# p2004dr/visual-slam

Hardware: AMD Instinct MI355X
Metric: frames/sec (extract+match+pose) at 640×480, 2000 ORB, 1/2/4/8 MI355X (higher is better)
Workload: dtype u8

## Files before the change

include/vslam_amd.h:

```cpp
#ifndef VSLAM_AMD_H
#define VSLAM_AMD_H

#include <stddef.h>
#include <stdint.h>

#ifdef __cplusplus
extern "C" {
#endif

#define MO_ABI_VERSION 5
int mo_abi_version(void);

#define MO_OK 0
#define MO_ERR_ARG (-1)
#define MO_ERR_HIP (-2)
#define MO_ERR_CAPACITY (-3)
#define MO_ERR_UNSUPPORTED (-4)

#define MO_ORDER_LIBSTDCXX 0
#define MO_ORDER_MSVC 1

typedef struct mo_ctx mo_ctx;

typedef struct {
// ... 198 lines not shown

int mo_dev_status(mo_ctx*, int32_t flags[4]);

int mo_stage_times(mo_ctx*, const char*** names, float* ms, int cap);
int mo_stage_times_back(mo_ctx*, int back, const char*** names, float* ms, int cap);

int mo_host_times(mo_ctx*, double us[4]);
int mo_set_host_timing(mo_ctx*, int on);

int mo_dbg_pyramid_level(mo_ctx*, const mo_orb_params*, const uint8_t* gray, int w, int h, int level, int blurred,
                         uint8_t* out , int* lw, int* lh);
int mo_dbg_fast_level(mo_ctx*, const mo_orb_params*, const uint8_t* gray, int w, int h, int level,
                      int32_t* xys , int cap, int* n);
int mo_dbg_min_eigen(mo_ctx*, const uint8_t* gray, int w, int h, float* eig );
int mo_dbg_set_poison(mo_ctx*, int byte );
int mo_dbg_retain_best(mo_ctx*, const float* resp, int n, int n_points, int select_order, int32_t* order, int* n_out);

#ifdef __cplusplus
}
#endif
#endif
```

visual-slam_amd/csrc/api.hip:

```cpp
#include <algorithm>
#include <cmath>
#include <cstring>
#include <vector>

#include "common.h"

static inline int* host_flags(mo_ctx* c) { return mo_host_flags(c); }

extern "C" int mo_set_host_timing(mo_ctx* c, int on) {
    if (!c) return MO_ERR_ARG;
    c->host_timing = on != 0;
    return MO_OK;
}

extern "C" int mo_host_times(mo_ctx* c, double us[4]) {
    if (!c || !us) return MO_ERR_ARG;
    for (int i = 0; i < 4; i++) us[i] = c->host_us[i];
    return MO_OK;
}

static bool grow_fin_slots(mo_ctx* c, int levels);

static int check_flags(mo_ctx* c) {
    int f[4] = {0, 0, 0, 0};
// ... 21 lines not shown
                   mo_keypoint* d_kps, uint8_t* d_desc, int cap, int32_t* d_counts, int host_call) {
    int rc = mo_build_plan(c, p, w, h, batch);
    if (rc) return rc;
    if (cap < 1) return mo_fail(c, MO_ERR_ARG, "cap must be >= 1");
    c->flags_cur = host_call ? host_flags(c) : c->d_flags;
    if (host_call == 1) HIPCHK(c, hipMemsetAsync(host_flags(c), 0, 4 * sizeof(int), c->stream));
    if (c->poison >= 0) {
        HIPCHK(c, hipMemsetAsync(c->d_pyr, c->poison, (size_t)c->batch_alloc * c->plan.pyr_stride, c->stream));
        HIPCHK(c, hipMemsetAsync(c->d_blur, c->poison, (size_t)c->batch_alloc * c->plan.blur_stride, c->stream));
    }
    if (host_call) mo_stage_mark(c, "h2d");
    else mo_stage_begin(c);
    const int blur_margin = (c->plan.edge_threshold - 19) & ~3, pyr_margin = std::max(blur_margin - 4, 0);
    if (batch <= MO_FS_MAX_BATCH && c->fs_ok) {
        if ((rc = orb_launch_front_single(c, d_gray, batch, d_desc != nullptr))) return rc;
        mo_stage_mark(c, "pyramid");
        if (d_desc) mo_stage_mark(c, "blur");
    } else {
        if ((rc = orb_launch_pyramid(c, d_gray, batch, c->plan.nlevels, pyr_margin))) return rc;
        mo_stage_mark(c, "pyramid");
        if (d_desc) {
            if ((rc = orb_launch_blur(c, d_gray, batch, c->plan.nlevels, blur_margin))) return rc;
            mo_stage_mark(c, "blur");
        }
    }
    if ((rc = orb_launch_fast(c, d_gray, batch))) return rc;
    mo_stage_mark(c, "fast_nms");
    if ((rc = orb_launch_select(c, d_gray, batch))) return rc;
    mo_stage_mark(c, "select_harris");
    if ((rc = orb_launch_describe(c, d_gray, batch, d_kps, d_desc, cap, d_counts))) return rc;
// ... 359 lines not shown
    const int nk = hn[65];
    if (hn[64] != n || nk < 0 || nk > n) return mo_fail(c, MO_ERR_HIP, "grid corner counts disagree between host and device");
    *n_xy = n; *n_kept = nk;
    std::memcpy(kept_idx, ho + (o_kept - o_out), (size_t)nk * sizeof(int32_t));
    std::memcpy(desc, ho + (o_desc - o_out), (size_t)nk * 32);
    mo_slot_commit(c, slot, nk);
    return MO_OK;
}

extern "C" int mo_dbg_set_poison(mo_ctx* c, int byte) {
    if (!c) return MO_ERR_ARG;
    c->poison = byte < 0 ? -1 : (byte & 255);
    return MO_OK;
}

extern "C" int mo_dbg_min_eigen(mo_ctx* c, const uint8_t* gray, int w, int h, float* eig) {
    if (!c) return MO_ERR_ARG;
    HIPCHK(c, hipSetDevice(c->device));
    return gftt_run(c, gray, w, h, w, 1, 64, nullptr, nullptr, eig);
}

extern "C" int mo_match_knn2_ratio(mo_ctx* c, const uint8_t* q, int nq, const uint8_t* t, int nt, const double* ratio,
                                   int batch, int32_t* train_idx, int32_t* dist, uint8_t* pass) {
    if (!c) return MO_ERR_ARG;
    if (nq < 0 || nt < 0 || batch < 1) return mo_fail(c, MO_ERR_ARG, "bad sizes");
    if (nq == 0) return MO_OK;
    if (!q || !train_idx || !dist || !pass || (nt > 0 && !t)) return mo_fail(c, MO_ERR_ARG, "NULL argument");
    HIPCHK(c, hipSetDevice(c->device));
    HostClock clk(c);
    size_t qb = (size_t)batch * nq * 32, tb = (size_t)batch * std::max(nt, 1) * 32, n = (size_t)batch * nq;
// ... 336 lines not shown
        mo_stage_mark(c, "two_view");
    }
    return MO_OK;
}

extern "C" int mo_dbg_pyramid_level(mo_ctx* c, const mo_orb_params* p, const uint8_t* gray, int w, int h, int level,
                                    int blurred, uint8_t* out, int* lw, int* lh) {
    if (!c) return MO_ERR_ARG;
    HIPCHK(c, hipSetDevice(c->device));
    int rc = mo_build_plan(c, p, w, h, 1);
    if (rc) return rc;
    if (level < 0 || level >= c->plan.nlevels) return mo_fail(c, MO_ERR_ARG, "level out of range");
    const uint8_t* d_gray = nullptr;
    if ((rc = stage_images(c, gray, w, h, w, 1, 1, &d_gray))) return rc;
    const bool fused = (blurred & 2) != 0;
    blurred &= 1;
    if (fused) {
        if (!c->fs_ok) return mo_fail(c, MO_ERR_UNSUPPORTED, std::string("the single-frame pyramid kernel does not cover this geometry: ") + c->fs_why);
        HIPCHK(c, hipMemsetAsync(c->d_pyr, 0xA5, (size_t)c->plan.pyr_stride, c->stream));
        HIPCHK(c, hipMemsetAsync(c->d_blur, 0xA5, (size_t)c->plan.blur_stride, c->stream));
        if ((rc = orb_launch_front_single(c, d_gray, 1, 1))) return rc;
    } else if ((rc = orb_launch_pyramid(c, d_gray, 1, c->plan.nlevels, 0))) return rc;
    const LevelInfo& v = c->plan.lv[level];
    *lw = v.w; *lh = v.h;
    if (blurred) {
        if (!fused && (rc = orb_launch_blur(c, d_gray, 1, c->plan.nlevels, 0))) return rc;
        HIPCHK(c, hipMemcpy2DAsync(out, v.w, c->d_blur + v.boff, v.bpitch, v.w, v.h, hipMemcpyDeviceToHost, c->stream));
    } else {
        const uint8_t* src = level == 0 ? d_gray : c->d_pyr + v.off;
        HIPCHK(c, hipMemcpy2DAsync(out, v.w, src, v.pitch, v.w, v.h, hipMemcpyDeviceToHost, c->stream));
    }
    HIPCHK(c, hipStreamSynchronize(c->stream));
    return MO_OK;
}

extern "C" int mo_dbg_fast_level(mo_ctx* c, const mo_orb_params* p, const uint8_t* gray, int w, int h, int level,
                                 int32_t* xys, int cap, int* n) {
    if (!c) return MO_ERR_ARG;
    HIPCHK(c, hipSetDevice(c->device));
    int rc = mo_build_plan(c, p, w, h, 1);
    if (rc) return rc;
// ... 44 lines not shown
```

visual-slam_amd/csrc/common.h:

```cpp
#pragma once
#include <hip/hip_runtime.h>
#include <chrono>
#include <stdint.h>
#include <string>
#include <vector>

#include "../../include/vslam_amd.h"

#define MO_MAX_LEVELS 12
#define MO_HALF_PATCH 15
#define MO_STRIP_ROWS 8
#ifndef MO_STRIP_ROWS_LATENCY
#define MO_STRIP_ROWS_LATENCY 2
#endif
#define SEL_MAXSTRIPS 2047

struct LevelInfo {
    int w, h, pitch;
    int off;
    int bpitch, boff;
    float scale;
    int quota;
    int bx0, by0, bw, bh;
    uint32_t inv_bw;
    int strip_rows;
    int nstrips;
    int strip_cap;
    int strip_base;
    int cand_off;
    int cand_cap;
// ... 55 lines not shown

    uint8_t* d_in = nullptr;       size_t d_in_bytes = 0;
    uint8_t* d_gray = nullptr;     size_t d_gray_bytes = 0;
    uint8_t* d_pyr = nullptr;
    uint8_t* d_blur = nullptr;
    uint32_t* d_cand = nullptr;
    int* d_strip_cnt = nullptr;
    uint64_t* d_scratch = nullptr;
    size_t scratch_stride = 0;
    FinalKp* d_fin = nullptr;
    int* d_fin_cnt = nullptr;
    uint32_t* d_tile_tab[2] = {nullptr, nullptr};
    int tile_cum[2][MO_MAX_LEVELS + 1] = {};
    int tile_margin = 0;
    uint32_t* d_fs_tab = nullptr; int fs_tiles = 0, fs_stride = 0, fs_lds = 0; bool fs_ok = false; int fs_geom[10] = {}; const char* fs_why = "";
    uint32_t* d_strip_tab = nullptr; int n_strip_tab = 0;
    uint32_t* d_dtile_tab = nullptr; int n_dtiles = 0, dtile_icw_off = 0;
    int* d_dtodo = nullptr; size_t dtodo_bytes = 0;
    int* d_flags = nullptr;
    int* flags_cur = nullptr;
    unsigned lds_attr_done = 0;
    mo_keypoint* d_kps = nullptr; uint8_t* d_desc = nullptr; int* d_counts = nullptr; int out_cap = 0, out_batch = 0;
    mo_keypoint* d_slot_kps = nullptr; uint8_t* d_slot_desc = nullptr; int32_t* d_slot_cnt = nullptr; int32_t* d_slot_ids = nullptr;
    int slot_cap = 0, slot_cur = -1;
    uint64_t slot_token[MO_RESULT_SLOTS] = {}; int slot_n[MO_RESULT_SLOTS] = {}; uint64_t token_next = 1, last_token = 0;
    bool host_timing = false;
    uint8_t* d_mq = nullptr; uint8_t* d_mt = nullptr; int32_t* d_midx = nullptr; int32_t* d_mdist = nullptr;
    uint8_t* d_mpass = nullptr; size_t m_q_bytes = 0, m_t_bytes = 0, m_n = 0;
    uint2* d_match_part = nullptr; size_t match_part_bytes = 0;
    void* d_tv = nullptr; size_t tv_bytes = 0;
// ... 56 lines not shown
uint64_t mo_slot_commit(mo_ctx* c, int slot, int n);
uint8_t* mo_stage_dev(mo_ctx* c);
void mo_copy_out_launch(mo_ctx* c, const void* d_src, void* h_dst_dev, size_t bytes);

void mo_stage_begin(mo_ctx* c);
void mo_stage_mark(mo_ctx* c, const char* name);

int mo_build_plan(mo_ctx* c, const mo_orb_params* p, int w, int h, int batch);

int orb_launch_gray(mo_ctx* c, const uint8_t* d_bgr, int w, int h, int batch, uint8_t* d_gray);
int orb_launch_ingest(mo_ctx* c, const uint8_t* src_mapped, int w, int h, int ch, uint8_t* d_gray, int* flags_clear);
int orb_launch_pyramid(mo_ctx* c, const uint8_t* d_gray, int batch, int nlevels, int margin);
#define MO_FS_MAX_BATCH 2
int fs_build(mo_ctx* c);
int orb_launch_front_single(mo_ctx* c, const uint8_t* d_gray, int batch, int want_blur);
void mo_linear_coeffs(int srcsize, int dstsize, std::vector<int>& ofs, std::vector<int>& c1);
int orb_launch_blur(mo_ctx* c, const uint8_t* d_gray, int batch, int nlevels, int margin);
int orb_launch_fast(mo_ctx* c, const uint8_t* d_gray, int batch, int level_lo = 0, int level_hi = MO_MAX_LEVELS);
int orb_launch_select(mo_ctx* c, const uint8_t* d_gray, int batch, int level_lo = 0, int level_hi = MO_MAX_LEVELS);
int orb_launch_describe(mo_ctx* c, const uint8_t* d_gray, int batch, mo_keypoint* d_kps, uint8_t* d_desc, int cap,
                        int* d_counts);
int orb_launch_describe_given(mo_ctx* c, const uint8_t* d_gray, const mo_keypoint* d_kps, int n, uint8_t* d_desc, const int* d_n = nullptr,
                              int batch = 1, int n_stride = 0);
int gftt_records_launch(mo_ctx* c, const float* d_xy, int* d_cell_n, int per_cell, int w, int h, int edge, mo_keypoint* d_rec,
                        int32_t* d_kept, int rec_stride, int32_t* d_counts_out, int batch, int32_t* d_kbase = nullptr);
int orb_launch_describe_cells(mo_ctx* c, const mo_keypoint* d_kps, const int32_t* d_kbase, uint8_t* d_desc, int cap, int batch);
int orb_launch_retain_probe(mo_ctx* c, const float* d_resp, int n, int n_points, int order, int32_t* d_order,
                            int* d_nout);
int match_launch_pairs(mo_ctx* c, const uint8_t* d_q, const uint8_t* d_t, size_t q_stride, size_t t_stride,
                       const int32_t* d_counts, const int32_t* d_qf, const int32_t* d_tf, int nq_fixed, int nt_fixed,
// ... 32 lines not shown
```

visual-slam_amd/csrc/ctx.hip:

```cpp
#include <algorithm>
#include <cmath>
#include <cstring>
#include <vector>

#include <cstdlib>

#include "common.h"

int mo_fail(mo_ctx* c, int code, const std::string& msg) {
    if (c) c->err = msg;
    return code;
}

static std::string g_create_err;

static inline int cv_round_f(float v) { return (int)lrintf(v); }
static inline int cv_round_d(double v) { return (int)lrint(v); }
static inline int align_up(int v, int a) { return (v + a - 1) / a * a; }

extern "C" int mo_abi_version(void) { return MO_ABI_VERSION; }

extern "C" int mo_device_count(void) {
    int n = 0;
    if (hipGetDeviceCount(&n) != hipSuccess) return 0;
// ... 36 lines not shown
    hipMemset(c->d_flags, 0, 8 * sizeof(int));
    c->flags_cur = c->d_flags;
    return c;
}

static void free_plan_buffers(mo_ctx* c) {
    for (int L = 0; L < MO_MAX_LEVELS; L++) {
        ResizeTab& t = c->rtab[L];
        if (t.xpk) hipFree(t.xpk);
        t = ResizeTab();
    }
    void* bufs[] = {c->d_pyr, c->d_blur, c->d_cand, c->d_strip_cnt, c->d_scratch, c->d_fin, c->d_fin_cnt, c->d_tile_tab[0], c->d_tile_tab[1], c->d_strip_tab, c->d_dtile_tab};
    c->d_dtile_tab = nullptr; c->n_dtiles = 0;
    if (c->d_fs_tab) hipFree(c->d_fs_tab);
    c->d_fs_tab = nullptr; c->fs_ok = false;
    for (void* b : bufs) if (b) hipFree(b);
    c->d_tile_tab[0] = c->d_tile_tab[1] = nullptr; c->d_strip_tab = nullptr; c->n_strip_tab = 0;
    c->d_pyr = c->d_blur = nullptr; c->d_cand = nullptr; c->d_strip_cnt = nullptr; c->d_scratch = nullptr;
    c->d_fin = nullptr; c->d_fin_cnt = nullptr;
    c->batch_alloc = 0;
    c->plan_valid = false;
}

extern "C" void mo_destroy(mo_ctx* c) {
    if (!c) return;
    hipSetDevice(c->device);
    hipDeviceSynchronize();
    mo_comm_destroy(c);
    free_plan_buffers(c);
    void* bufs[] = {c->d_in, c->d_gray, c->d_flags, c->d_kps, c->d_desc, c->d_counts, c->d_mq, c->d_mt,
// ... 241 lines not shown
    }

    size_t B = (size_t)batch;
    HIPCHK(c, hipMalloc((void**)&c->d_pyr, B * P.pyr_stride));
    HIPCHK(c, hipMalloc((void**)&c->d_blur, B * P.blur_stride));
    HIPCHK(c, hipMalloc((void**)&c->d_cand, B * P.cand_stride * sizeof(uint32_t)));
    HIPCHK(c, hipMalloc((void**)&c->d_strip_cnt, B * P.strips_per_frame * sizeof(int)));
    HIPCHK(c, hipMalloc((void**)&c->d_scratch, B * c->scratch_stride * sizeof(uint64_t)));
    if (hipMalloc((void**)&c->d_fin, B * P.fin_stride * sizeof(FinalKp)) != hipSuccess)
        return mo_fail(c, MO_ERR_HIP, "hipMalloc of the final-keypoint slots failed: " + std::to_string(B * P.fin_stride * sizeof(FinalKp)) +
                                          " bytes (" + std::to_string(batch) + " frames x " + std::to_string(P.fin_stride) + " slots; slots grow with response ties)");
    HIPCHK(c, hipMalloc((void**)&c->d_fin_cnt, B * MO_MAX_LEVELS * sizeof(int)));
    {
        const int rc_fs = fs_build(c);
        if (rc_fs) return rc_fs;
    }
    c->batch_alloc = batch;
    c->plan_params = *p;
    c->plan_valid = true;
    c->fin_slack_dirty = false;
    return MO_OK;
}
```

visual-slam_amd/csrc/orb_kernels.hip:

```cpp
#include <cstring>

#include "common.h"
#include "select_replay.h"

__constant__ __attribute__((aligned(16))) int8_t c_pattern[256 * 4] = {
#include "orb_pattern.inc"
};

#define WAVE 64

__device__ __forceinline__ int reflect101(int p, int len) {
    if (len == 1) return 0;
    while (p < 0 || p >= len) p = p < 0 ? -p : 2 * len - 2 - p;
    return p;
}

__device__ __forceinline__ void xcd_map(uint32_t lin, uint32_t per, uint32_t inv_per, uint32_t batch, int& frame, int& item) {
    const uint32_t b8 = batch & ~7u, cut = per * b8;
    const bool head = lin < cut;
    const uint32_t n = head ? lin >> 3 : lin - cut;
    const uint32_t q = inv_per ? __umulhi(n, inv_per) : n;
    item = (int)(n - q * per);
    frame = (int)(head ? (lin & 7u) + 8u * q : b8 + q);
}

__device__ __forceinline__ const uint8_t* level_ptr(const Plan& P, int L, const uint8_t* gray, const uint8_t* pyr,
                                                    int frame) {
    return L == 0 ? gray + (size_t)frame * P.w * P.h : pyr + (size_t)frame * P.pyr_stride + P.lv[L].off;
}

__global__ void k_gray(const uint8_t* __restrict__ bgr, uint8_t* __restrict__ gray, size_t npx) {
    size_t i = (size_t)blockIdx.x * blockDim.x + threadIdx.x;
    if (i >= npx) return;
    int b = bgr[3 * i], g = bgr[3 * i + 1], r = bgr[3 * i + 2];
    gray[i] = (uint8_t)((b * 3735 + g * 19235 + r * 9798 + (1 << 14)) >> 15);
}

int orb_launch_gray(mo_ctx* c, const uint8_t* d_bgr, int w, int h, int batch, uint8_t* d_gray) {
// ... 1470 lines not shown
```

visual-slam_amd/vslam_amd/__init__.py:

```python
import ctypes as C
import os
import weakref

import numpy as np

_PKG_ROOT = os.path.dirname(os.path.dirname(os.path.abspath(__file__)))
LIB_PATH = os.environ.get("VSLAM_AMD_LIB") or os.path.join(_PKG_ROOT, "libvslam_amd.so")

MO_OK, MO_ERR_ARG, MO_ERR_HIP, MO_ERR_CAPACITY, MO_ERR_UNSUPPORTED = 0, -1, -2, -3, -4
ABI_VERSION = 5
ORDER_LIBSTDCXX, ORDER_MSVC = 0, 1

KP_DTYPE = np.dtype([("x", "<f4"), ("y", "<f4"), ("size", "<f4"), ("angle", "<f4"), ("response", "<f4"),
                     ("octave", "<i4"), ("class_id", "<i4")])
assert KP_DTYPE.itemsize == 28


class NativeUnavailable(RuntimeError):
    pass


class NativeError(RuntimeError):
    def __init__(self, code, msg):
        super().__init__("libvslam_amd error %d: %s" % (code, msg))
# ... 61 lines not shown
SIGNATURES = {
    "mo_create": (_vp, [_i, _i, _i, _i]),
    "mo_destroy": (None, [_vp]),
    "mo_last_error": (C.c_char_p, [_vp]),
    "mo_set_stream": (_i, [_vp, _vp]),
    "mo_set_stream_null": (_i, [_vp]),
    "mo_sync": (_i, [_vp]),
    "mo_device_count": (_i, []),
    "mo_abi_version": (_i, []),
    "mo_orb_detect_compute": (_i, [_vp, _vp, _vp, _i, _i, _i, _i, _i, _vp, _vp, _i, _vp]),
    "mo_orb_compute": (_i, [_vp, _vp, _vp, _i, _i, _i, _i, _vp, _i, _vp, _vp, _vp]),
    "mo_orb_grid_good_features": (_i, [_vp, _vp, _i, _i, _i, _i, _i, _vp, _vp]),
    "mo_orb_grid_detect_compute": (_i, [_vp, _vp, _vp, _i, _i, _i, _i, _i, _vp, _vp, _vp, _vp, _vp]),
    "mo_dbg_min_eigen": (_i, [_vp, _vp, _i, _i, _vp]),
    "mo_dbg_set_poison": (_i, [_vp, _i]),
    "mo_undistort": (_i, [_vp, _vp, _i, _i, _i, _i, _vp, _vp, _vp]),
    "mo_dev_undistort": (_i, [_vp, _vp, _i, _i, _i, _i, _vp, _vp, _vp]),
    "mo_match_knn2_ratio": (_i, [_vp, _vp, _i, _vp, _i, _vp, _i, _vp, _vp, _vp]),
    "mo_init_two_view": (_i, [_vp, _vp, _vp, _i, _vp, _d, _d, _i, C.c_uint64, _vp, _vp, _vp, _vp, _vp, _vp, _vp]),
    "mo_recover_pose": (_i, [_vp, _vp, _vp, _vp, _i, _vp, _vp, _vp, _vp, _vp, _vp, _vp]),
    "mo_find_fundamental": (_i, [_vp, _vp, _vp, _i, _d, _d, _i, C.c_uint64, _vp, _vp, _vp]),
    "mo_track_pair": (_i, [_vp, _vp, _i, _vp, _vp, _i, _vp, _i, _i, _d, _d, _vp, _d, _i, C.c_uint64, _vp, _vp, _vp, _vp, _vp, _vp, _vp,
                           _vp]),
    "mo_triangulate_points": (_i, [_vp, _vp, _vp, _vp, _vp, _i, _vp]),
    "mo_dev_frontend_batch": (_i, [_vp, _vp, _vp]),
    "mo_dev_orb_detect_compute": (_i, [_vp, _vp, _vp, _i, _i, _i, _vp, _vp, _i, _vp]),
    "mo_dev_match_pairs": (_i, [_vp, _vp, _vp, _i, _vp, _vp, _i, _d, _vp, _vp, _vp]),
    "mo_dev_status": (_i, [_vp, _vp]),
    "mo_stream_create": (_vp, [_vp, _vp, _vp]),
    "mo_stream_destroy": (None, [_vp]),
# ... 436 lines not shown
```

Before: 108,200.

## Add banded batched fused pyramid+blur kernel keeping levels in LDS

Adds a new kernel that builds the whole image pyramid and Gaussian blur for each horizontal band of a frame inside LDS. Each workgroup handles one band and recomputes halo rows across levels, replacing the separate per-level resize and blur launches for large batches. A heuristic (fb_pays) turns it on only when there are enough workgroups to keep the CUs busy. The cost is redundant halo computation and one workgroup per CU because of the large LDS footprint.

```diff
diff --git a/include/vslam_amd.h b/include/vslam_amd.h
--- a/include/vslam_amd.h
+++ b/include/vslam_amd.h
@@ -236,6 +236,7 @@
                       int32_t* xys , int cap, int* n);
 int mo_dbg_min_eigen(mo_ctx*, const uint8_t* gray, int w, int h, float* eig );
 int mo_dbg_set_poison(mo_ctx*, int byte );
+int mo_dbg_set_front_batch(mo_ctx*, int on);
 int mo_dbg_retain_best(mo_ctx*, const float* resp, int n, int n_points, int select_order, int32_t* order, int* n_out);
 
 #ifdef __cplusplus
diff --git a/profiles/front_batch_model.py b/profiles/front_batch_model.py
--- /dev/null
+++ b/profiles/front_batch_model.py
@@ -0,0 +1,100 @@
+#!/usr/bin/env python3
+import argparse
+import math
+
+CUS, SIMDS, GHZ = 256, 4, 2.4
+FAST, SLOW = 2.26, 4.5
+LDS_CU = 160 * 1024
+RESIZE_Q = (22, 28)
+BLUR_ROW = (5, 14)
+BLUR_OUT = (6, 16)
+K = 8
+MAX_RECOMPUTE = 0.4
+
+
+def cv_round(x):
+    return int(math.floor(x + 0.5))
+
+
+def linear_ofs(src, dst):
+    scale = src / dst
+    ofs = []
+    for v in range(dst):
+        f = scale * (v + 0.5) - 0.5
+        i = math.floor(f)
+        ofs.append(0 if i < 0 else min(i, src - 1))
+    return ofs
+
+
+def reflect(p, n):
+    while p < 0 or p >= n:
+        p = -p if p < 0 else 2 * n - 2 - p
+    return p
+
+
+def model(w, h, nl, sf, nb, batch, budget):
+    W = [cv_round(w / sf ** L) for L in range(nl)]
+    H = [cv_round(h / sf ** L) for L in range(nl)]
+    yo = [None] + [linear_ofs(H[L - 1], H[L]) for L in range(1, nl)]
+    pw = [((x + 3) & ~3) + 12 for x in W]
+    qr = [((x + 6) >> 2) + 1 for x in W]
+    xtot = sum(4 * qr[L] for L in range(1, nl))
+    own_rows = [0] * nl
+    eys = []
+    ht = hb = 0
+    for b in range(nb):
+        ey = [None] * nl
+        for L in range(nl - 1, -1, -1):
+            o0, o1 = b * H[L] // nb, (b + 1) * H[L] // nb
+            rows = [reflect(y, H[L]) for y in range(o0 - 3, o1 + 3)]
+            lo, hi = min(rows), max(rows)
+            if L + 1 < nl:
+                n0, n1 = ey[L + 1]
+                lo = min(lo, yo[L + 1][n0]); hi = max(hi, min(yo[L + 1][n1 - 1] + 1, H[L] - 1))
+            ey[L] = (lo, hi + 1)
+            own_rows[L] += o1 - o0
+            if L == 0:
+                ht, hb = max(ht, o0 - lo), max(hb, hi + 1 - o1)
+        eys.append(ey)
+    ext_rows = [0] * nl
+    lds_max = 0
+    for b, ey in enumerate(eys):
+        o0, o1 = b * H[0] // nb, (b + 1) * H[0] // nb
+        ey[0] = (max(o0 - ht, 0), min(o1 + hb, H[0]))
+        for L in range(nl):
+            ext_rows[L] += ey[L][1] - ey[L][0]
+        buf = [max((pw[L] * (ey[L][1] - ey[L][0]) + 15) & ~15 for L in range(par, nl, 2)) for par in (0, 1)]
+        ytot = (sum(ey[L][1] - ey[L][0] for L in range(1, nl)) + 3) & ~3
+        lds_max = max(lds_max, sum(buf) + 4 * (xtot + ytot))
+    wg_cu = LDS_CU // lds_max if lds_max <= budget else 0
+    wg_cu = min(wg_cu, 1)
+    quads = lambda L, rows: rows * qr[L] if L else rows * (pw[L] - 12) // 4
+    res_tasks = sum(quads(L, ext_rows[L]) for L in range(1, nl)) / 64
+    bq = lambda L, rows: rows * (pw[L] - 12) // 4
+    blur_rows = sum(bq(L, own_rows[L] * (K + 6) // K) for L in range(nl)) / 64
+    blur_out = sum(bq(L, own_rows[L]) for L in range(nl)) / 64
+    cyc = sum(n * c for (n, c) in [(RESIZE_Q[0] * res_tasks, FAST), (RESIZE_Q[1] * res_tasks, SLOW),
+                                   (BLUR_ROW[0] * blur_rows, FAST), (BLUR_ROW[1] * blur_rows, SLOW),
+                                   (BLUR_OUT[0] * blur_out, FAST), (BLUR_OUT[1] * blur_out, SLOW)])
+    issue_ms = cyc * batch / (CUS * SIMDS) / (GHZ * 1e6)
+    read0 = ext_rows[0] * w
+    wbytes = sum(W[L] * H[L] for L in range(1, nl)) + sum(W[L] * H[L] for L in range(nl))
+    return dict(nb=nb, band0=h // nb, halo0=(ht, hb), recompute=[round(ext_rows[L] / H[L] - 1, 3) for L in range(nl)], lds_kb=round(lds_max / 1024, 1),
+                wg_per_cu=wg_cu, mb_per_step=round((read0 + wbytes) * batch / 1e6, 1), hbm_ms=round((read0 + wbytes) * batch / 6.29e9, 3),
+                issue_ms=round(issue_ms, 3), wgs=nb * batch)
+
+
+if __name__ == "__main__":
+    ap = argparse.ArgumentParser()
+    ap.add_argument("--w", type=int, default=640); ap.add_argument("--h", type=int, default=480)
+    ap.add_argument("--levels", type=int, default=8); ap.add_argument("--scale", type=float, default=1.2)
+    ap.add_argument("--batch", type=int, default=256); ap.add_argument("--budget-kb", type=float, default=158)
+    a = ap.parse_args()
+    budget = a.budget_kb * 1024
+    taken = False
+    for nb in (2, 3, 4, 5, 6, 8, 10, 12, 16, 21):
+        m = model(a.w, a.h, a.levels, a.scale, nb, a.batch, budget)
+        fits = m["lds_kb"] * 1024 <= budget
+        mark = ("  <- fb_build" if m["recompute"][0] <= MAX_RECOMPUTE else "  <- fits, refused by fb_build (halo bound)") if not taken and fits else ""
+        taken = taken or bool(mark)
+        print(m, mark)
diff --git a/visual-slam_amd/csrc/api.hip b/visual-slam_amd/csrc/api.hip
--- a/visual-slam_amd/csrc/api.hip
+++ b/visual-slam_amd/csrc/api.hip
@@ -59,6 +59,10 @@
     const int blur_margin = (c->plan.edge_threshold - 19) & ~3, pyr_margin = std::max(blur_margin - 4, 0);
     if (batch <= MO_FS_MAX_BATCH && c->fs_ok) {
         if ((rc = orb_launch_front_single(c, d_gray, batch, d_desc != nullptr))) return rc;
+        mo_stage_mark(c, "pyramid");
+        if (d_desc) mo_stage_mark(c, "blur");
+    } else if (c->fb_ok && (c->fb_mode == 2 || (c->fb_mode == 1 && fb_pays(c, batch)))) {
+        if ((rc = orb_launch_front_batch(c, d_gray, batch, d_desc != nullptr, pyr_margin, blur_margin))) return rc;
         mo_stage_mark(c, "pyramid");
         if (d_desc) mo_stage_mark(c, "blur");
     } else {
@@ -448,6 +452,13 @@
     return MO_OK;
 }
 
+extern "C" int mo_dbg_set_front_batch(mo_ctx* c, int on) {
+    if (!c) return MO_ERR_ARG;
+    if (on < 0 || on > 2) return mo_fail(c, MO_ERR_ARG, "mo_dbg_set_front_batch: on must be 0, 1 or 2");
+    c->fb_mode = on;
+    return MO_OK;
+}
+
 extern "C" int mo_dbg_min_eigen(mo_ctx* c, const uint8_t* gray, int w, int h, float* eig) {
     if (!c) return MO_ERR_ARG;
     HIPCHK(c, hipSetDevice(c->device));
@@ -814,8 +825,14 @@
     const uint8_t* d_gray = nullptr;
     if ((rc = stage_images(c, gray, w, h, w, 1, 1, &d_gray))) return rc;
     const bool fused = (blurred & 2) != 0;
+    const bool banded = (blurred & 4) != 0;
     blurred &= 1;
-    if (fused) {
+    if (banded) {
+        if (!c->fb_ok) return mo_fail(c, MO_ERR_UNSUPPORTED, std::string("the batched pyramid kernel does not cover this geometry: ") + c->fb_why);
+        HIPCHK(c, hipMemsetAsync(c->d_pyr, 0xA5, (size_t)c->plan.pyr_stride, c->stream));
+        HIPCHK(c, hipMemsetAsync(c->d_blur, 0xA5, (size_t)c->plan.blur_stride, c->stream));
+        if ((rc = orb_launch_front_batch(c, d_gray, 1, 1, 0, 0))) return rc;
+    } else if (fused) {
         if (!c->fs_ok) return mo_fail(c, MO_ERR_UNSUPPORTED, std::string("the single-frame pyramid kernel does not cover this geometry: ") + c->fs_why);
         HIPCHK(c, hipMemsetAsync(c->d_pyr, 0xA5, (size_t)c->plan.pyr_stride, c->stream));
         HIPCHK(c, hipMemsetAsync(c->d_blur, 0xA5, (size_t)c->plan.blur_stride, c->stream));
@@ -824,7 +841,7 @@
     const LevelInfo& v = c->plan.lv[level];
     *lw = v.w; *lh = v.h;
     if (blurred) {
-        if (!fused && (rc = orb_launch_blur(c, d_gray, 1, c->plan.nlevels, 0))) return rc;
+        if (!fused && !banded && (rc = orb_launch_blur(c, d_gray, 1, c->plan.nlevels, 0))) return rc;
         HIPCHK(c, hipMemcpy2DAsync(out, v.w, c->d_blur + v.boff, v.bpitch, v.w, v.h, hipMemcpyDeviceToHost, c->stream));
     } else {
         const uint8_t* src = level == 0 ? d_gray : c->d_pyr + v.off;
diff --git a/visual-slam_amd/csrc/common.h b/visual-slam_amd/csrc/common.h
--- a/visual-slam_amd/csrc/common.h
+++ b/visual-slam_amd/csrc/common.h
@@ -14,6 +14,15 @@
 #define MO_STRIP_ROWS_LATENCY 2
 #endif
 #define SEL_MAXSTRIPS 2047
+
+static __device__ __forceinline__ void xcd_map(uint32_t lin, uint32_t per, uint32_t inv_per, uint32_t batch, int& frame, int& item) {
+    const uint32_t b8 = batch & ~7u, cut = per * b8;
+    const bool head = lin < cut;
+    const uint32_t n = head ? lin >> 3 : lin - cut;
+    const uint32_t q = inv_per ? __umulhi(n, inv_per) : n;
+    item = (int)(n - q * per);
+    frame = (int)(head ? (lin & 7u) + 8u * q : b8 + q);
+}
 
 struct LevelInfo {
     int w, h, pitch;
@@ -99,6 +108,9 @@
     int tile_cum[2][MO_MAX_LEVELS + 1] = {};
     int tile_margin = 0;
     uint32_t* d_fs_tab = nullptr; int fs_tiles = 0, fs_stride = 0, fs_lds = 0; bool fs_ok = false; int fs_geom[10] = {}; const char* fs_why = "";
+    uint32_t* d_fb_tab = nullptr; bool fb_ok = false; int fb_geom[72] = {}; const char* fb_why = "";
+    int fb_cus = 1;
+    int fb_mode = 1;
     uint32_t* d_strip_tab = nullptr; int n_strip_tab = 0;
     uint32_t* d_dtile_tab = nullptr; int n_dtiles = 0, dtile_icw_off = 0;
     int* d_dtodo = nullptr; size_t dtodo_bytes = 0;
@@ -185,6 +197,9 @@
 #define MO_FS_MAX_BATCH 2
 int fs_build(mo_ctx* c);
 int orb_launch_front_single(mo_ctx* c, const uint8_t* d_gray, int batch, int want_blur);
+int fb_build(mo_ctx* c);
+int orb_launch_front_batch(mo_ctx* c, const uint8_t* d_gray, int batch, int want_blur, int pyr_margin, int blur_margin);
+bool fb_pays(const mo_ctx* c, int batch);
 void mo_linear_coeffs(int srcsize, int dstsize, std::vector<int>& ofs, std::vector<int>& c1);
 int orb_launch_blur(mo_ctx* c, const uint8_t* d_gray, int batch, int nlevels, int margin);
 int orb_launch_fast(mo_ctx* c, const uint8_t* d_gray, int batch, int level_lo = 0, int level_hi = MO_MAX_LEVELS);
diff --git a/visual-slam_amd/csrc/ctx.hip b/visual-slam_amd/csrc/ctx.hip
--- a/visual-slam_amd/csrc/ctx.hip
+++ b/visual-slam_amd/csrc/ctx.hip
@@ -74,6 +74,8 @@
     c->d_dtile_tab = nullptr; c->n_dtiles = 0;
     if (c->d_fs_tab) hipFree(c->d_fs_tab);
     c->d_fs_tab = nullptr; c->fs_ok = false;
+    if (c->d_fb_tab) hipFree(c->d_fb_tab);
+    c->d_fb_tab = nullptr; c->fb_ok = false;
     for (void* b : bufs) if (b) hipFree(b);
     c->d_tile_tab[0] = c->d_tile_tab[1] = nullptr; c->d_strip_tab = nullptr; c->n_strip_tab = 0;
     c->d_pyr = c->d_blur = nullptr; c->d_cand = nullptr; c->d_strip_cnt = nullptr; c->d_scratch = nullptr;
@@ -345,6 +347,8 @@
     {
         const int rc_fs = fs_build(c);
         if (rc_fs) return rc_fs;
+        const int rc_fb = fb_build(c);
+        if (rc_fb) return rc_fb;
     }
     c->batch_alloc = batch;
     c->plan_params = *p;
diff --git a/visual-slam_amd/csrc/front_batch.hip b/visual-slam_amd/csrc/front_batch.hip
--- /dev/null
+++ b/visual-slam_amd/csrc/front_batch.hip
@@ -0,0 +1,398 @@
+#include "common.h"
+
+#include <algorithm>
+#include <cstring>
+#include <vector>
+
+#ifndef FB_NT
+#define FB_NT 1024
+#endif
+#ifndef FB_K
+#define FB_K 8
+#endif
+#define FB_STAGE_U 4
+#define FB_BOX_INTS 5
+#define FB_HDR_INTS (MO_MAX_LEVELS * FB_BOX_INTS)
+#ifndef FB_MAX_RECOMPUTE
+#define FB_MAX_RECOMPUTE 0.4
+#endif
+#define FB_MIN_ROUNDS 4
+#define FB_MAX_IDLE 0.05
+#ifndef FB_LDS_BUDGET
+#define FB_LDS_BUDGET (158 * 1024)
+#endif
+
+struct FbGeom {
+    int nb;
+    uint32_t inv_per;
+    int stride;
+    int ht, hb;
+    int xtot;
+    int ye_base;
+    int buf[2];
+    int lds;
+    int xe_off[MO_MAX_LEVELS];
+    int qw[MO_MAX_LEVELS];
+    int pitch[MO_MAX_LEVELS];
+    uint32_t inv_qw[MO_MAX_LEVELS];
+    int nrg[MO_MAX_LEVELS];
+};
+
+static inline __host__ __device__ int fb_reflect(int p, int len) {
+    if (len == 1) return 0;
+    while (p < 0 || p >= len) p = p < 0 ? -p : 2 * len - 2 - p;
+    return p;
+}
+
+static int fb_no(mo_ctx* c, const char* why) { c->fb_why = why; return MO_OK; }
+
+int fb_build(mo_ctx* c) {
+    c->fb_ok = false; c->fb_why = "";
+    if (c->d_fb_tab) { hipFree(c->d_fb_tab); c->d_fb_tab = nullptr; }
+    const Plan& P = c->plan;
+    const int nl = P.nlevels;
+    if (nl < 2) return fb_no(c, "one level: nothing to chain");
+    FbGeom G = {};
+    std::vector<std::vector<int>> xo(nl), xc(nl), yo(nl), yc(nl);
+    int xtot = 0;
+    for (int L = 0; L < nl; L++) {
+        const int W = P.lv[L].w;
+        G.qw[L] = L == 0 ? ((W + 3) & ~3) >> 2 : ((W + 6) >> 2) + 2;
+        if (G.qw[L] > FB_NT) return fb_no(c, "level wider than 4 columns per thread");
+        G.pitch[L] = ((W + 3) & ~3) + 12;
+        G.inv_qw[L] = G.qw[L] > 1 ? 0xFFFFFFFFu / (uint32_t)G.qw[L] + 1u : 0u;
+        G.nrg[L] = FB_NT / G.qw[L];
+        if (L == 0) continue;
+        if (!c->rtab[L].two_pass_ok) return fb_no(c, "4 output columns need more than an 8-byte source window");
+        mo_linear_coeffs(P.lv[L - 1].w, W, xo[L], xc[L]);
+        mo_linear_coeffs(P.lv[L - 1].h, P.lv[L].h, yo[L], yc[L]);
+        G.xe_off[L] = xtot;
+        xtot += 4 * G.qw[L];
+    }
+    G.xtot = xtot;
+    const int Htop = P.lv[nl - 1].h;
+    std::vector<uint32_t> all;
+    size_t lds = 0;
+    for (int nb = 1; nb <= Htop; nb++) {
+        std::vector<std::vector<int>> ey(nb, std::vector<int>(nl)), eh(nb, std::vector<int>(nl)), oy(nb, std::vector<int>(nl)),
+            oy1(nb, std::vector<int>(nl));
+        int ht = 0, hb = 0;
+        for (int b = 0; b < nb; b++)
+            for (int L = nl - 1; L >= 0; L--) {
+                const int H = P.lv[L].h;
+                const int o0 = (int)((long long)b * H / nb), o1 = (int)((long long)(b + 1) * H / nb);
+                int lo = H, hi = -1;
+                for (int y = o0 - 3; y < o1 + 3; y++) { const int r = fb_reflect(y, H); lo = std::min(lo, r); hi = std::max(hi, r); }
+                if (L + 1 < nl) {
+                    const int n0 = ey[b][L + 1], n1 = n0 + eh[b][L + 1] - 1;
+                    lo = std::min(lo, yo[L + 1][n0]); hi = std::max(hi, std::min(yo[L + 1][n1] + 1, H - 1));
+                }
+                ey[b][L] = lo; eh[b][L] = hi + 1 - lo; oy[b][L] = o0; oy1[b][L] = o1;
+                if (L == 0) { ht = std::max(ht, o0 - lo); hb = std::max(hb, hi + 1 - o1); }
+            }
+        for (int b = 0; b < nb; b++) {
+            const int e0 = std::max(oy[b][0] - ht, 0), e1 = std::min(oy1[b][0] + hb, P.h);
+            ey[b][0] = e0; eh[b][0] = e1 - e0;
+        }
+        int ytot = 0;
+        for (int b = 0; b < nb; b++) {
+            int t = 0;
+            for (int L = 1; L < nl; L++) t += eh[b][L];
+            ytot = std::max(ytot, t);
+        }
+        ytot = (ytot + 3) & ~3;
+        size_t buf[2] = {0, 0};
+        for (int b = 0; b < nb; b++)
+            for (int L = 0; L < nl; L++) buf[L & 1] = std::max(buf[L & 1], ((size_t)G.pitch[L] * eh[b][L] + 15) & ~(size_t)15);
+        const size_t need = (size_t)(xtot + ytot) * 4 + buf[0] + buf[1];
+        if (need > FB_LDS_BUDGET && nb < Htop) continue;
+        if (need > FB_LDS_BUDGET) return fb_no(c, "no band height fits the LDS budget");
+        {
+            long long rows0 = 0;
+            for (int b = 0; b < nb; b++) rows0 += eh[b][0];
+            if ((double)rows0 / P.h - 1.0 > FB_MAX_RECOMPUTE) return fb_no(c, "the bands that fit the LDS recompute too much halo (the per-level kernels are faster)");
+        }
+        G.nb = nb; G.ht = ht; G.hb = hb; G.ye_base = xtot;
+        G.buf[0] = (xtot + ytot) * 4; G.buf[1] = G.buf[0] + (int)buf[0];
+        G.stride = FB_HDR_INTS + ytot;
+        G.inv_per = nb > 1 ? 0xFFFFFFFFu / (uint32_t)nb + 1u : 0u;
+        lds = need;
+        all.assign((size_t)nb * G.stride + xtot, 0u);
+        for (int b = 0; b < nb; b++) {
+            uint32_t* blob = &all[(size_t)b * G.stride];
+            int yoff = 0;
+            for (int L = 0; L < nl; L++) {
+                uint32_t* h = blob + L * FB_BOX_INTS;
+                h[0] = (uint32_t)ey[b][L]; h[1] = (uint32_t)eh[b][L]; h[2] = (uint32_t)oy[b][L]; h[3] = (uint32_t)oy1[b][L]; h[4] = (uint32_t)yoff;
+                const int H = P.lv[L].h;
+                for (int y = oy[b][L] - 3; y < oy1[b][L] + 3; y++) {
+                    const int r = fb_reflect(y, H);
+                    if (r < ey[b][L] || r >= ey[b][L] + eh[b][L]) return fb_no(c, "blur rows outside the level's box");
+                }
+                if (L == 0) continue;
+                const int SH = P.lv[L - 1].h;
+                for (int r = 0; r < eh[b][L]; r++) {
+                    const int j = ey[b][L] + r, o = yo[L][j], o1 = std::min(o + 1, SH - 1), rel = o - ey[b][L - 1];
+                    if (rel < 0 || rel + (o1 - o) >= eh[b][L - 1] || rel > 0x7FFF) return fb_no(c, "row source index outside the previous level's box");
+                    blob[FB_HDR_INTS + yoff + r] = (uint32_t)rel | ((uint32_t)(o1 - o) << 15) | ((uint32_t)yc[L][j] << 16);
+                }
+                yoff += eh[b][L];
+            }
+        }
+        for (int L = 1; L < nl; L++) {
+            const int W = P.lv[L].w, SW = P.lv[L - 1].w;
+            if (4 + 4 * (G.qw[L] - 2) + 4 > G.pitch[L]) return fb_no(c, "resize quads past the level's LDS row");
+            for (int i = 0; i < 4 * G.qw[L]; i += 4) {
+                int lo = SW, hi = 0;
+                for (int k = 0; k < 4; k++) {
+                    const int j = fb_reflect(i + k - 4, W), o = xo[L][j], o1 = std::min(o + 1, SW - 1);
+                    all[(size_t)nb * G.stride + G.xe_off[L] + i + k] = (uint32_t)o | ((uint32_t)(o1 - o) << 15) | ((uint32_t)xc[L][j] << 16);
+                    lo = std::min(lo, o); hi = std::max(hi, o1);
+                }
+                if (hi - lo > 7) return fb_no(c, "4 output columns need more than an 8-byte source window");
+                if (4 + (lo & ~3) + 12 > G.pitch[L - 1]) return fb_no(c, "source window past the previous level's row");
+            }
+        }
+        break;
+    }
+    if (G.nb == 0) return fb_no(c, "no band height fits the LDS budget");
+    HIPCHK(c, hipMalloc((void**)&c->d_fb_tab, all.size() * sizeof(uint32_t)));
+    HIPCHK(c, hipMemcpy(c->d_fb_tab, all.data(), all.size() * sizeof(uint32_t), hipMemcpyHostToDevice));
+    G.lds = (int)lds;
+    static_assert(sizeof(FbGeom) <= sizeof(c->fb_geom) && offsetof(FbGeom, nb) == 0, "FbGeom and mo_ctx::fb_geom (fb_pays reads nb)");
+    std::memcpy(c->fb_geom, &G, sizeof(G));
+    int cus = 0;
+    HIPCHK(c, hipDeviceGetAttribute(&cus, hipDeviceAttributeMultiprocessorCount, c->device));
+    c->fb_cus = std::max(cus, 1);
+    c->fb_ok = true;
+    return MO_OK;
+}
+
+typedef unsigned short fb_u16x2 __attribute__((ext_vector_type(2)));
+__device__ __forceinline__ uint32_t fb_udot2(uint32_t a, uint32_t b, uint32_t c) {
+    return __builtin_amdgcn_udot2(__builtin_bit_cast(fb_u16x2, a), __builtin_bit_cast(fb_u16x2, b), c, false);
+}
+__device__ __forceinline__ uint32_t fb_hi16_pair_sat_u8(uint32_t a, uint32_t b) {
+    uint32_t d;
+    asm("v_sat_pk_u8_i16 %0, %1" : "=v"(d) : "v"(__builtin_amdgcn_perm(b, a, 0x07060302u)));
+    return d;
+}
+
+__device__ __forceinline__ void fb_cover(int len, int m, int tile, int& org, int& end) {
+    const int span = max(len - 2 * m, 1);
+    org = m;
+    end = min(len, m + (span + tile - 1) / tile * tile);
+}
+
+__device__ __forceinline__ void fb_pads(uint8_t* A, int pitch, int eh, int W, int tid) {
+    const int hi = ((W + 3) & ~3) + 3;
+    for (int r = tid; r < eh; r += FB_NT) {
+        uint8_t* row = A + r * pitch + 4;
+        for (int k = -3; k < 0; k++) row[k] = row[fb_reflect(k, W)];
+        for (int k = W; k <= hi; k++) row[k] = row[fb_reflect(k, W)];
+    }
+}
+
+__global__ __launch_bounds__(FB_NT) void k_front_batch(Plan P, FbGeom G, const uint32_t* __restrict__ tab, const uint8_t* __restrict__ gray,
+                                                       uint8_t* __restrict__ pyr, uint8_t* __restrict__ blur, int want_blur, int pyr_margin,
+                                                       int blur_margin) {
+    extern __shared__ __attribute__((aligned(16))) uint8_t lds[];
+    __shared__ int s_hdr[FB_HDR_INTS];
+    const int tid = threadIdx.x, nl = P.nlevels;
+    int frame, band;
+    xcd_map(blockIdx.x + gridDim.x * blockIdx.y, gridDim.x, G.inv_per, gridDim.y, frame, band);
+    const uint32_t* blob = tab + (size_t)band * G.stride;
+    uint32_t* s_xe = (uint32_t*)lds;
+    uint32_t* s_ye = s_xe + G.ye_base;
+    {
+        if (tid < FB_HDR_INTS) s_hdr[tid] = (int)blob[tid];
+        for (int i = tid; i < G.stride - FB_HDR_INTS; i += FB_NT) s_ye[i] = blob[FB_HDR_INTS + i];
+        const uint32_t* xe = tab + (size_t)G.nb * G.stride;
+        for (int i = tid; i < G.xtot; i += FB_NT) s_xe[i] = xe[i];
+        const int oy0 = (int)((long long)band * P.h / G.nb), oy1 = (int)((long long)(band + 1) * P.h / G.nb);
+        const int ey0 = max(oy0 - G.ht, 0), eh = min(oy1 + G.hb, P.h) - ey0;
+        const int qw = G.qw[0], pitch = G.pitch[0];
+        const int rg = G.inv_qw[0] ? (int)__umulhi((uint32_t)tid, G.inv_qw[0]) : tid, q = tid - rg * qw, nrg = G.nrg[0];
+        const uint8_t* g = gray + (size_t)frame * P.w * P.h + (size_t)ey0 * P.w;
+        const bool al = (P.w & 3) == 0 && (((size_t)gray) & 3) == 0;
+        uint8_t* A = lds + G.buf[0];
+        if (rg < nrg) {
+            for (int r0 = rg; r0 < eh; r0 += FB_STAGE_U * nrg) {
+                uint32_t v[FB_STAGE_U];
+#pragma unroll
+                for (int u = 0; u < FB_STAGE_U; u++) {
+                    const int r = r0 + u * nrg;
+                    v[u] = 0;
+                    if (r < eh) {
+                        const uint8_t* row = g + (size_t)r * P.w;
+                        if (al) v[u] = *(const uint32_t*)(row + 4 * q);
+                        else {
+#pragma unroll
+                            for (int k = 0; k < 4; k++) v[u] |= (uint32_t)row[min(4 * q + k, P.w - 1)] << (8 * k);
+                        }
+                    }
+                }
+#pragma unroll
+                for (int u = 0; u < FB_STAGE_U; u++) {
+                    const int r = r0 + u * nrg;
+                    if (r < eh) *(uint32_t*)(A + r * pitch + 4 + 4 * q) = v[u];
+                }
+            }
+        }
+    }
+    __syncthreads();
+    if (want_blur) {
+        fb_pads(lds + G.buf[0], G.pitch[0], s_hdr[1], P.w, tid);
+        __syncthreads();
+    }
+    const uint32_t g0 = P.gk[0], g1 = P.gk[1], g2 = P.gk[2], g3 = P.gk[3], g6 = P.gk[6];
+    const uint32_t ta = g0 | (g1 << 8) | (g2 << 16) | (g3 << 24), tb = g2 | (g1 << 8) | (g0 << 16);
+    const uint32_t gp[3] = {g0 | (g1 << 16), g2 | (g3 << 16), (uint32_t)P.gk[4] | ((uint32_t)P.gk[5] << 16)};
+    for (int L = 0; L < nl; L++) {
+        const int* hb = s_hdr + L * FB_BOX_INTS;
+        const LevelInfo lv = P.lv[L];
+        const int qw = G.qw[L], pitch = G.pitch[L];
+        uint8_t* A = lds + G.buf[L & 1];
+        const int ey0 = hb[0], eh = hb[1], oy0 = hb[2], oy1 = hb[3];
+        if (L > 0) {
+            const int rg = G.inv_qw[L] ? (int)__umulhi((uint32_t)tid, G.inv_qw[L]) : tid, q = tid - rg * qw, nrg = G.nrg[L];
+            const int spitch = G.pitch[L - 1];
+            const uint8_t* S = lds + G.buf[(L - 1) & 1];
+            if (rg < nrg) {
+                const uint4 xe = *(const uint4*)(s_xe + G.xe_off[L] + 4 * q);
+                const uint32_t xk[4] = {xe.x, xe.y, xe.z, xe.w};
+                const int ox0 = (int)min(min(xk[0] & 0x7FFFu, xk[1] & 0x7FFFu), min(xk[2] & 0x7FFFu, xk[3] & 0x7FFFu)), ab = ox0 & ~3;
+                const uint32_t sh8 = (uint32_t)(ox0 & 3);
+                uint32_t sel[4], coef[4];
+#pragma unroll
+                for (int k = 0; k < 4; k++) {
+                    const uint32_t a = (xk[k] & 0x7FFFu) - (uint32_t)ox0, b = a + ((xk[k] >> 15) & 1u), c1 = xk[k] >> 16;
+                    sel[k] = a | (b << 16) | 0x0C000C00u;
+                    coef[k] = (256u - c1) | (c1 << 16);
+                }
+                int porg, pend, prow0, prow1;
+                const int pm = (lv.w > 2 * pyr_margin + 8 && lv.h > 2 * pyr_margin + 8) ? pyr_margin : 0;
+                fb_cover(lv.w, pm, 64, porg, pend);
+                fb_cover(lv.h, pm, 64, prow0, prow1);
+                const int x = 4 * (q - 1);
+                const bool col_out = x >= porg && x < pend;
+                const int y_lo = max(oy0, prow0), y_hi = min(oy1, prow1);
+                uint8_t* dst = pyr + (size_t)frame * P.pyr_stride + lv.off;
+                const uint32_t* ye_l = s_ye + hb[4];
+                for (int r = rg; r < eh; r += 2 * nrg) {
+                    const int rb = min(r + nrg, eh - 1);
+                    const uint32_t e[2] = {ye_l[r], ye_l[rb]};
+                    uint32_t a[2][2][3];
+#pragma unroll
+                    for (int t = 0; t < 2; t++) {
+                        const uint8_t* r0 = S + (e[t] & 0x7FFFu) * spitch + 4 + ab;
+                        const uint8_t* r1 = r0 + ((e[t] >> 15) & 1u) * spitch;
+#pragma unroll
+                        for (int d = 0; d < 3; d++) { a[t][0][d] = ((const uint32_t*)r0)[d]; a[t][1][d] = ((const uint32_t*)r1)[d]; }
+                    }
+#pragma unroll
+                    for (int t = 0; t < 2; t++) {
+                        const uint32_t c1 = e[t] >> 16, cy = (256u - c1) | (c1 << 16);
+                        const uint32_t u0 = __builtin_amdgcn_alignbyte(a[t][0][1], a[t][0][0], sh8), u1 = __builtin_amdgcn_alignbyte(a[t][0][2], a[t][0][1], sh8);
+                        const uint32_t w0 = __builtin_amdgcn_alignbyte(a[t][1][1], a[t][1][0], sh8), w1 = __builtin_amdgcn_alignbyte(a[t][1][2], a[t][1][1], sh8);
+                        uint32_t v[4];
+#pragma unroll
+                        for (int k = 0; k < 4; k++) {
+                            const uint32_t h0 = fb_udot2(__builtin_amdgcn_perm(u1, u0, sel[k]), coef[k], 0u);
+                            const uint32_t h1 = fb_udot2(__builtin_amdgcn_perm(w1, w0, sel[k]), coef[k], 0u);
+                            v[k] = fb_udot2(h0 | (h1 << 16), cy, 32768u);
+                        }
+                        const uint32_t packed = __builtin_amdgcn_perm(v[1], v[0], 0x0C0C0602u) | (__builtin_amdgcn_perm(v[3], v[2], 0x0C0C0602u) << 16);
+                        const int rr = t ? rb : r;
+                        *(uint32_t*)(A + rr * pitch + 4 + x) = packed;
+                        const int y = ey0 + rr;
+                        if (col_out && y >= y_lo && y < y_hi) *(uint32_t*)(dst + (size_t)y * lv.pitch + x) = packed;
+                    }
+                }
+            }
+            __syncthreads();
+        }
+        if (!want_blur) continue;
+        {
+            int bx0, bx1, by0, by1;
+            fb_cover(lv.w, blur_margin, 64, bx0, bx1);
+            fb_cover(lv.h, blur_margin, 58, by0, by1);
+            const int r_lo = max(oy0, by0), r_hi = min(oy1, by1);
+            const int q0 = bx0 >> 2, nq = ((bx1 + 3) >> 2) - q0;
+            if (r_hi > r_lo && nq > 0) {
+                const uint32_t inv = nq > 1 ? 0xFFFFFFFFu / (uint32_t)nq + 1u : 0u;
+                const int rg = inv ? (int)__umulhi((uint32_t)tid, inv) : tid, q = tid - rg * nq, nrg = FB_NT / nq;
+                const int nch = (r_hi - r_lo + FB_K - 1) / FB_K;
+                const int H = lv.h, x0 = 4 * (q0 + q);
+                uint8_t* out = blur + (size_t)frame * P.blur_stride + lv.boff + x0;
+                if (rg < nrg) {
+                    for (int ch = rg; ch < nch; ch += nrg) {
+                        const int yb = r_lo + ch * FB_K;
+                        uint32_t acc[FB_K][4], prev[4] = {0, 0, 0, 0};
+#pragma unroll
+                        for (int j = 0; j < FB_K; j++)
+#pragma unroll
+                            for (int k = 0; k < 4; k++) acc[j][k] = 1u << 15;
+#pragma unroll
+                        for (int i = 0; i < FB_K + 6; i++) {
+                            int y = yb - 3 + i;
+                            y = y < 0 ? -y : y;
+                            y = y >= H ? 2 * H - 2 - y : y;
+                            const int ly = min(max(y - ey0, 0), eh - 1);
+                            const uint8_t* row = A + ly * pitch;
+                            const uint32_t* pw = (const uint32_t*)(row + x0);
+                            const uint32_t w0 = pw[0], w1 = pw[1], w2 = pw[2];
+                            uint32_t rs[4];
+                            rs[0] = __builtin_amdgcn_udot4(__builtin_amdgcn_alignbyte(w1, w0, 1), ta, __builtin_amdgcn_udot4(__builtin_amdgcn_alignbyte(w2, w1, 1), tb, 0, false), false);
+                            rs[1] = __builtin_amdgcn_udot4(__builtin_amdgcn_alignbyte(w1, w0, 2), ta, __builtin_amdgcn_udot4(__builtin_amdgcn_alignbyte(w2, w1, 2), tb, 0, false), false);
+                            rs[2] = __builtin_amdgcn_udot4(__builtin_amdgcn_alignbyte(w1, w0, 3), ta, __builtin_amdgcn_udot4(__builtin_amdgcn_alignbyte(w2, w1, 3), tb, 0, false), false);
+                            rs[3] = __builtin_amdgcn_udot4(w1, ta, __builtin_amdgcn_udot4(w2, tb, 0, false), false);
+#pragma unroll
+                            for (int p = 0; p < 3; p++) {
+                                const int j = i - 1 - 2 * p;
+                                if (i >= 1 && j >= 0 && j < FB_K) {
+#pragma unroll
+                                    for (int k = 0; k < 4; k++) acc[j][k] = fb_udot2(prev[k] | (rs[k] << 16), gp[p], acc[j][k]);
+                                }
+                            }
+                            if (i - 6 >= 0 && i - 6 < FB_K) {
+#pragma unroll
+                                for (int k = 0; k < 4; k++) acc[i - 6][k] += g6 * rs[k];
+                            }
+#pragma unroll
+                            for (int k = 0; k < 4; k++) prev[k] = rs[k];
+                        }
+#pragma unroll
+                        for (int j = 0; j < FB_K; j++) {
+                            const int y = yb + j;
+                            if (y < r_hi)
+                                *(uint32_t*)(out + (size_t)y * lv.bpitch) =
+                                    fb_hi16_pair_sat_u8(acc[j][0], acc[j][1]) | (fb_hi16_pair_sat_u8(acc[j][2], acc[j][3]) << 16);
+                        }
+                    }
+                }
+            }
+        }
+    }
+}
+
+bool fb_pays(const mo_ctx* c, int batch) {
+    if (!c->fb_ok) return false;
+    const long long wgs = (long long)c->fb_geom[0] * batch, rounds = (wgs + c->fb_cus - 1) / c->fb_cus;
+    return rounds >= FB_MIN_ROUNDS && (double)wgs >= (1.0 - FB_MAX_IDLE) * (double)(rounds * c->fb_cus);
+}
+
+int orb_launch_front_batch(mo_ctx* c, const uint8_t* d_gray, int batch, int want_blur, int pyr_margin, int blur_margin) {
+    if (!c->fb_ok || !c->d_fb_tab) return mo_fail(c, MO_ERR_ARG, "front_batch: no band table for this plan");
+    if ((pyr_margin | blur_margin) & 3) return mo_fail(c, MO_ERR_ARG, "front_batch: margins must be multiples of 4");
+    FbGeom G;
+    std::memcpy(&G, c->fb_geom, sizeof(G));
+    if (!(c->lds_attr_done & (1u << 16))) {
+        HIPCHK(c, hipFuncSetAttribute((const void*)k_front_batch, hipFuncAttributeMaxDynamicSharedMemorySize, FB_LDS_BUDGET));
+        c->lds_attr_done |= 1u << 16;
+    }
+    hipLaunchKernelGGL(k_front_batch, dim3((unsigned)G.nb, (unsigned)batch), dim3(FB_NT), (size_t)G.lds, c->stream, c->plan, G, c->d_fb_tab,
+                       d_gray, c->d_pyr, c->d_blur, want_blur, pyr_margin, blur_margin);
+    HIPCHK(c, hipGetLastError());
+    return MO_OK;
+}
diff --git a/visual-slam_amd/csrc/orb_kernels.hip b/visual-slam_amd/csrc/orb_kernels.hip
--- a/visual-slam_amd/csrc/orb_kernels.hip
+++ b/visual-slam_amd/csrc/orb_kernels.hip
@@ -13,15 +13,6 @@
     if (len == 1) return 0;
     while (p < 0 || p >= len) p = p < 0 ? -p : 2 * len - 2 - p;
     return p;
-}
-
-__device__ __forceinline__ void xcd_map(uint32_t lin, uint32_t per, uint32_t inv_per, uint32_t batch, int& frame, int& item) {
-    const uint32_t b8 = batch & ~7u, cut = per * b8;
-    const bool head = lin < cut;
-    const uint32_t n = head ? lin >> 3 : lin - cut;
-    const uint32_t q = inv_per ? __umulhi(n, inv_per) : n;
-    item = (int)(n - q * per);
-    frame = (int)(head ? (lin & 7u) + 8u * q : b8 + q);
 }
 
 __device__ __forceinline__ const uint8_t* level_ptr(const Plan& P, int L, const uint8_t* gray, const uint8_t* pyr,
diff --git a/visual-slam_amd/vslam_amd/__init__.py b/visual-slam_amd/vslam_amd/__init__.py
--- a/visual-slam_amd/vslam_amd/__init__.py
+++ b/visual-slam_amd/vslam_amd/__init__.py
@@ -99,6 +99,7 @@
     "mo_orb_grid_detect_compute": (_i, [_vp, _vp, _vp, _i, _i, _i, _i, _i, _vp, _vp, _vp, _vp, _vp]),
     "mo_dbg_min_eigen": (_i, [_vp, _vp, _i, _i, _vp]),
     "mo_dbg_set_poison": (_i, [_vp, _i]),
+    "mo_dbg_set_front_batch": (_i, [_vp, _i]),
     "mo_undistort": (_i, [_vp, _vp, _i, _i, _i, _i, _vp, _vp, _vp]),
     "mo_dev_undistort": (_i, [_vp, _vp, _i, _i, _i, _i, _vp, _vp, _vp]),
     "mo_match_knn2_ratio": (_i, [_vp, _vp, _i, _vp, _i, _vp, _i, _vp, _vp, _vp]),
```

Measured after the change: 109,300 (median of 6 runs). 1.01x the previous value.
